# georgegrosu1/torch-admm-deconv

Measured on AMD Instinct MI355X. Metric: ADMM iterations/sec, batch-64 1024x1024x3, 50 iters; rel-L2 vs CPU ref, higher is better.
Workload: dtype f32

## Files before the change

### torch-admm-deconv_amd/csrc/admm_capi.hip

```cpp
#include <hip/hip_runtime.h>

#include <cstdlib>
#include <cstring>
#include <mutex>
#include <string>
#include <type_traits>
#include <vector>

#include "gcol_mm.hpp"
#include "knobs.hpp"
#include "mixed_capi.hpp"
#include "odd_capi.hpp"
#include "admm_tv.h"

using namespace admm;

namespace {

thread_local std::string g_err;

int fail(int code, const std::string& msg) {
    g_err = msg;
    return code;
}
// ... 204 lines not shown
    } while (0)

template <class K> int set_lds(K kern, size_t bytes) {
    if (bytes > 64 * 1024) {
        hipError_t e = hipFuncSetAttribute(reinterpret_cast<const void*>(kern),
                                           hipFuncAttributeMaxDynamicSharedMemorySize, (int)bytes);
        if (e != hipSuccess) return fail(ADMM_TV_EHIP, std::string("hipFuncSetAttribute: ") + hipGetErrorString(e));
    }
    return 0;
}

int launch_check(const char* what) {
    hipError_t e = hipGetLastError();
    if (e != hipSuccess) return fail(ADMM_TV_EHIP, std::string(what) + ": " + hipGetErrorString(e));
    return 0;
}

template <class T>
int bwd_scalars(double* part, int K, long long nstrips, long long spm, long long soff, const double* tpart, int ntp,
                int G, int g, const T* lam, const T* rho, T* glam, T* grho, hipStream_t s) {
    if (K < 1) return fail(ADMM_TV_EINVAL, "bwd_scalars: no iterations");
    hipLaunchKernelGGL(k_bwd_iter_sums, dim3((unsigned)K), dim3(256), 0, s, part, nstrips, spm, soff, tpart, ntp, G, g);
    if (int e = launch_check("k_bwd_iter_sums")) return e;
    hipLaunchKernelGGL(k_bwd_scalars<T>, dim3(1), dim3(256), 0, s, (const double*)part, K, nstrips, 1LL, soff,
                       (const double*)nullptr, ntp, G, g, lam, rho, glam, grho);
    return launch_check("k_bwd_scalars");
}

template <int N> struct RowOps {
    using G = RowKernelGeom<N>;
    static unsigned blocks(long long items) { return (unsigned)((items + G::SG - 1) / G::SG); }

    static int r2c(const float* img, cf* spec, const cf* twW, long long rows, hipStream_t s, bool pl = false) {
        if (pl)
            hipLaunchKernelGGL((k_row_r2c<N, true>), dim3(blocks(rows)), dim3(G::NT), G::lds_bytes(), s, img, spec, twW, rows);
        else
            hipLaunchKernelGGL((k_row_r2c<N, false>), dim3(blocks(rows)), dim3(G::NT), G::lds_bytes(), s, img, spec, twW, rows);
        return launch_check("k_row_r2c");
    }
    static int c2r(const cf* spec, float* img, const cf* twW, long long rows, hipStream_t s, bool pl = false) {
        if (pl)
            hipLaunchKernelGGL((k_row_c2r<N, true>), dim3(blocks(rows)), dim3(G::NT), G::lds_bytes(), s, spec, img, twW, rows);
        else
            hipLaunchKernelGGL((k_row_c2r<N, false>), dim3(blocks(rows)), dim3(G::NT), G::lds_bytes(), s, spec, img, twW, rows);
        return launch_check("k_row_c2r");
    }
    static int pair(const float* img, float* out, long long rows, hipStream_t s) {
        hipLaunchKernelGGL(k_row_pair<N>, dim3(blocks(rows)), dim3(G::NT), 0, s, img, out, rows);
        return launch_check("k_row_pair");
    }
    template <bool ISO, bool FIRST, bool HIST, bool PL> static void pa(const PassAArgs& a, unsigned nb, hipStream_t s) {
        hipLaunchKernelGGL((k_pass_a<N, ISO, FIRST, HIST, PL>), dim3(nb), dim3(G::NT), G::lds_bytes(), s, a);
    }
    static int pass_a(const PassAArgs& a, bool iso, bool first, bool hist, hipStream_t s, bool pl = false) {
        const unsigned nb = blocks(a.nstrips);
        const int sel = (iso ? 4 : 0) | (first ? 2 : 0) | (hist ? 1 : 0);
        if (pl && !hist) {
            switch (sel) {
                case 0: pa<false, false, false, true>(a, nb, s); break;
                case 2: pa<false, true, false, true>(a, nb, s); break;
                case 4: pa<true, false, false, true>(a, nb, s); break;
                default: pa<true, true, false, true>(a, nb, s); break;
            }
            return launch_check("k_pass_a");
        }
        switch (sel) {
            case 0: pa<false, false, false, false>(a, nb, s); break;
            case 1: pa<false, false, true, false>(a, nb, s); break;
            case 2: pa<false, true, false, false>(a, nb, s); break;
            case 3: pa<false, true, true, false>(a, nb, s); break;
            case 4: pa<true, false, false, false>(a, nb, s); break;
            case 5: pa<true, false, true, false>(a, nb, s); break;
            case 6: pa<true, true, false, false>(a, nb, s); break;
            default: pa<true, true, true, false>(a, nb, s); break;
        }
        return launch_check("k_pass_a");
    }
    static int iso_norm(const IsoArgs& a, bool first, bool hist, hipStream_t s, bool pl = false) {
        const unsigned nb = blocks(a.nitems);
        if (first && pl)
            hipLaunchKernelGGL((k_iso_norm<N, true, false, true>), dim3(nb), dim3(G::NT), G::lds_bytes(), s, a);
        else if (first)
            hipLaunchKernelGGL((k_iso_norm<N, true, false, false>), dim3(nb), dim3(G::NT), G::lds_bytes(), s, a);
        else if (hist)
            hipLaunchKernelGGL((k_iso_norm<N, false, true, false>), dim3(nb), dim3(G::NT), G::lds_bytes(), s, a);
        else if (pl)
            hipLaunchKernelGGL((k_iso_norm<N, false, false, true>), dim3(nb), dim3(G::NT), G::lds_bytes(), s, a);
        else
            hipLaunchKernelGGL((k_iso_norm<N, false, false, false>), dim3(nb), dim3(G::NT), G::lds_bytes(), s, a);
        return launch_check("k_iso_norm");
    }
    template <bool ISO, bool LASTK, bool FIRSTK> static void bpa(const BwdArgs& a, unsigned nb, hipStream_t s) {
        using BG = BwdGeom<N>;
        hipLaunchKernelGGL((k_bwd_pass_a<N, ISO, LASTK, FIRSTK>), dim3(nb), dim3(BG::NT), BG::lds_bytes(), s, a);
    }
    static int bwd_pass_a(const BwdArgs& a, bool iso, bool lastk, bool firstk, hipStream_t s) {
        const unsigned nb = (unsigned)((a.nstrips + BwdGeom<N>::SG - 1) / BwdGeom<N>::SG);
        const int sel = (iso ? 4 : 0) | (lastk ? 2 : 0) | (firstk ? 1 : 0);
        switch (sel) {
            case 0: bpa<false, false, false>(a, nb, s); break;
            case 1: bpa<false, false, true>(a, nb, s); break;
            case 2: bpa<false, true, false>(a, nb, s); break;
            case 3: bpa<false, true, true>(a, nb, s); break;
            case 4: bpa<true, false, false>(a, nb, s); break;
            case 5: bpa<true, false, true>(a, nb, s); break;
            case 6: bpa<true, true, false>(a, nb, s); break;
            default: bpa<true, true, true>(a, nb, s); break;
        }
        return launch_check("k_bwd_pass_a");
// ... 1100 lines not shown
    {
        ProfScope ps(3, s);
        if (d.kh > 0) {
            float* bb = at<float>(ws, Lo.b);
            if (env_int("ADMM_MIXED_BGEN", 0)) {
                if (int e = gapply<float>(xin, bb, spec[0], Lo, ws, d, 1, s)) return e;
            } else {
                if (int e = hchk(admm_mixed::r2c(N, xin, spec[0], twW, rows, s), "k_row_r2c_m")) return e;
                if (int e = hchk(admm_mixed::pass_b_cm(H, spec[0], at<cf>(ws, Lo.mM), twH, N, P, s), "k_pass_b_m<cm>"))
                    return e;
                if (int e = hchk(admm_mixed::c2r(N, spec[0], bb, twW, rows, s), "k_row_c2r_m")) return e;
            }
            bimg = bb;
        }
        if (int e = hchk(admm_mixed::r2c(N, bimg, spec[0], twW, rows, s), "k_row_r2c_m")) return e;
    }
    const int R = strip_rows_mixed(H, rows, N);
    const int G = ngroups_of(d);
    const int gpm = Lo.ngroups / G;
    for (int g = 0; g < G; ++g) {
    const float* fcM = at<float>(ws, Lo.fcM) + (size_t)g * (2 * N + 1) * H;
    const float* lamg = lam + g;
    const float* rhog = rho + g;
    float* outg = out + (size_t)g * P * H * W;
    if (g > 0) {
        ProfScope ps(3, s);
        if (int e = hchk(admm_mixed::r2c(N, bimg, spec[0], twW, rows, s), "k_row_r2c_m")) return e;
    }
    int cur = 0, uin = 0;
    for (int it = 1; it <= d.maxit; ++it) {
        {
            ProfScope ps(1, s);
            if (int e = hchk(admm_mixed::pass_b(H, spec[cur], fcM, twH, N, P, s), "k_pass_b_m")) return e;
        }
        if (it == d.maxit) {
            ProfScope ps(3, s);
            if (int e = hchk(admm_mixed::c2r(N, spec[cur], outg, twW, rows, s), "k_row_c2r_m")) return e;
            if (!train) break;
        }
        const bool first = it == 1;
        const float *uxi, *uyi, *nprev = nullptr;
        float *uxo, *uyo;
        if (train) {
            uxi = first ? nullptr : ha(it - 1, 0);
            uyi = first ? nullptr : ha(it - 1, 1);
            uxo = ha(it, 0);
            uyo = ha(it, 1);
            if (d.iso && !first) nprev = hn(it - 1);
        } else {
            uxi = u[2 * uin];
            uyi = u[2 * uin + 1];
            uxo = u[2 * (1 - uin)];
            uyo = u[2 * (1 - uin) + 1];
        }
        const float* nsq = nullptr;
        if (d.iso) {
            ProfScope ps(2, s);
            float* nout = train ? hn(it) : at<float>(ws, Lo.nsq);
            IsoArgs ia{spec[cur], uxi, uyi, nprev, lamg, rhog, at<float>(ws, Lo.part), twW, (int)P, H, Lo.ppg,
                       (long long)gpm * H, P};
            if (int e = hchk(admm_mixed::iso_norm(N, ia, first, train, s), "k_iso_norm_m")) return e;
            const long long n4 = 2LL * H * W / 4;
            hipLaunchKernelGGL(k_iso_reduce, dim3((unsigned)((n4 + 255) / 256)), dim3(256), 0, s, at<float4>(ws, Lo.part),
                               reinterpret_cast<float4*>(nout), gpm, n4);
            if (int e = launch_check("k_iso_reduce")) return e;
            allreduce(d, nout, 2ull * H * W, s);
            nsq = nout;
        }
        {
            ProfScope ps(0, s);
            PassAArgs pa{spec[cur], spec[1 - cur], bimg, uxi, uyi, uxo, uyo, nsq, nprev, lamg, rhog, twW, H, R,
                         rows / R, P, 0};
            if (int e = hchk(admm_mixed::pass_a(N, pa, d.iso != 0, first, train, s), "k_pass_a_m")) return e;
        }
        cur = 1 - cur;
        uin = 1 - uin;
    }
    }
    return 0;
}

int run_forward(const admm_tv_desc& d, const float* xin, const float* kern, const float* lam, const float* rho,
                float* out, void* ws, size_t ws_bytes, void* hist, hipStream_t s) {
    const Layout Lo = make_layout(d);
    if (!ws || ws_bytes < Lo.total || (reinterpret_cast<uintptr_t>(ws) % kAlign) != 0)
        return fail(ADMM_TV_EWORKSPACE, "workspace too small or not 256-byte aligned");
    if (Lo.tr && !hist && d.maxit > 0) {
        const long long P = d.B * d.C;
        const int H = (int)d.H, W = (int)d.W;
        float* xT = at<float>(ws, Lo.xT);
        float* oT = at<float>(ws, Lo.oT);
        float* kT = d.kh > 0 ? at<float>(ws, Lo.kT) : nullptr;
        {
            ProfScope ps(3, s);
            hipError_t e = admm_odd::transpose(xin, xT, H, W, P, s);
            if (e == hipSuccess && kT) e = admm_odd::transpose(kern, kT, d.kh, d.kw, 1, s);
            if (e != hipSuccess) return fail(ADMM_TV_EHIP, std::string("k_transpose: ") + hipGetErrorString(e));
        }
        const admm_tv_desc dT = transposed(d);
        if (int e = run_forward(dT, xT, kT, lam, rho, oT, at<char>(ws, Lo.tws), ws_bytes - Lo.tws, nullptr, s)) return e;
        ProfScope ps(3, s);
        const hipError_t e = admm_odd::transpose(oT, out, W, H, P, s);
        return e == hipSuccess ? 0 : fail(ADMM_TV_EHIP, std::string("k_transpose: ") + hipGetErrorString(e));
    }
    const int G = ngroups_of(d);
    const long long Pm = d.B * d.C, P = G * Pm;
// ... 13 lines not shown
                allreduce(d, at<float>(ws, Lo.nsq), n, s);
            }
        return 0;
    }
    if (int e = setup(d, Lo, ws, kern, rho, s)) return e;
    if (Lo.mixed && (!hist || Lo.mixed_train)) return run_forward_mixed(d, Lo, xin, lam, rho, out, ws, hist, s);
    if (Lo.gen) return run_forward_gen(d, Lo, xin, lam, rho, out, ws, hist, s);
    cf* twW = at<cf>(ws, Lo.twW);
    cf* twH = at<cf>(ws, Lo.twH);
    float* fcT = at<float>(ws, Lo.fcT);
    cf* mT = at<cf>(ws, Lo.mT);
    cf* spec[2] = {at<cf>(ws, Lo.spec[0]), at<cf>(ws, Lo.spec[1])};
    float* u[4] = {at<float>(ws, Lo.u[0]), at<float>(ws, Lo.u[1]), at<float>(ws, Lo.u[2]), at<float>(ws, Lo.u[3])};
    const bool train = hist != nullptr;
    const Hist Hs = make_hist(d);
    auto ha = [&](int k, int comp) -> float* {
        return reinterpret_cast<float*>(static_cast<char*>(hist) + (size_t)(2 * (k - 1) + comp) * Hs.a_slot);
    };
    auto hn = [&](int k) -> float* {
        return reinterpret_cast<float*>(static_cast<char*>(hist) + Hs.n_off + (size_t)(k - 1) * Hs.n_slot);
    };
    const bool keep_t = train && Hs.keep_t;
    auto ht = [&](int k) -> cf* {
        return reinterpret_cast<cf*>(static_cast<char*>(hist) + Hs.t_off + (size_t)(k - 1) * Hs.t_slot);
    };

    const bool pl = !train && env_int("ADMM_PL", (d.iso || W < 1024) ? 1 : 0) != 0;

    const float* bimg = xin;
    if (d.kh > 0) {
        ProfScope ps(3, s);
        float* bb = at<float>(ws, Lo.b);
        if (int e = psf_transpose_into(d, Lo, ws, xin, bb, spec[0], 1, s, pl)) return e;
        bimg = bb;
    } else if (pl) {
        ProfScope ps(3, s);
        float* bb = at<float>(ws, Lo.b);
        if (int e = with_row(N, [&](auto ops) { return decltype(ops)::pair(xin, bb, Pm * H, s); })) return e;
        bimg = bb;
    }
    for (int g = 0; g < G; ++g) {
        ProfScope ps(3, s);
        cf* t0 = (keep_t ? ht(1) : spec[0]) + (size_t)g * Pm * H * N;
        int e = with_row(N, [&](auto ops) { return decltype(ops)::r2c(bimg, t0, twW, Pm * H, s, pl); });
        if (e) return e;
    }
    auto solve_planes = [&](long long p0, long long np, long long ppm, hipStream_t st) -> int {
    const size_t so = (size_t)p0 * H * N, io = (size_t)p0 * H * W;
    cf* cspec[2] = {spec[0] + so, spec[1] + so};
    const long long crows = np * H;
    const float* cb = bimg + io;
    float* cout = out + io;
    const int R = strip_rows(H, N, crows, !d.iso && !hist);

    int cur = 0, uin = 0;
    for (int it = 1; it <= d.maxit; ++it) {
        {
            ProfScope ps(1, st);
            const cf* tin = keep_t ? ht(it) : cspec[cur];
            if (int e = pass_b_oop(H, tin, cspec[cur], fcT, mT, twH, N, (int)np, 0, st, (int)ppm)) return e;
        }
        if (it == d.maxit) {
            ProfScope ps(3, st);
            int e = with_row(N, [&](auto ops) { return decltype(ops)::c2r(cspec[cur], cout, twW, crows, st); });
            if (e) return e;
            if (!train) break;
        }
        const bool first = (it == 1);
        const float *uxi, *uyi, *nprev = nullptr;
        float *uxo, *uyo;
        if (train) {
            uxi = first ? nullptr : ha(it - 1, 0);
            uyi = first ? nullptr : ha(it - 1, 1);
            uxo = ha(it, 0);
            uyo = ha(it, 1);
            if (d.iso && !first) nprev = hn(it - 1);
        } else {
            uxi = u[2 * uin] + io;
            uyi = u[2 * uin + 1] + io;
            uxo = u[2 * (1 - uin)] + io;
            uyo = u[2 * (1 - uin) + 1] + io;
        }
        const float* nsq = nullptr;
        if (d.iso) {
            ProfScope ps(2, st);
            float* nout = train ? hn(it) : at<float>(ws, Lo.nsq);
            IsoArgs ia{cspec[cur], uxi, uyi, nprev, lam, rho, at<float>(ws, Lo.part), twW, (int)P, H, Lo.ppg,
                       (long long)Lo.ngroups * H, Pm};
            int e = with_row(N, [&](auto ops) { return decltype(ops)::iso_norm(ia, first, train, st, pl); });
            if (e) return e;
            const long long n4 = 2LL * H * W / 4;
            const int gpm = Lo.ngroups / G;
            for (int g = 0; g < G; ++g) {
                hipLaunchKernelGGL(k_iso_reduce, dim3((unsigned)((n4 + 255) / 256)), dim3(256), 0, st,
                                   at<float4>(ws, Lo.part) + (size_t)g * gpm * n4,
                                   reinterpret_cast<float4*>(nout) + (size_t)g * n4, gpm, n4);
                if ((e = launch_check("k_iso_reduce"))) return e;
            }
            allreduce(d, nout, (size_t)G * 2 * H * W, st);
            nsq = nout;
        }
        {
            ProfScope ps(0, st);
            cf* tout = (keep_t && it < d.maxit) ? ht(it + 1) : cspec[1 - cur];
            PassAArgs pa{cspec[cur], tout, cb, uxi, uyi, uxo, uyo, nsq, nprev, lam, rho, twW, H, R, crows / R, ppm,
                         env_int("ADMM_PASSA_REV", 0)};
            int e = with_row(N, [&](auto ops) { return decltype(ops)::pass_a(pa, d.iso != 0, first, train, st, pl); });
            if (e) return e;
        }
        cur = 1 - cur;
        uin = 1 - uin;
    }
    return 0;
    };
    return solve_planes(0, P, Pm, s);
}

struct BwdLayout {
    Layout f;
    size_t abar[4], bbar, part, tpart, q, xpart, aacc, zacc, total;
    long long nstrips;
    int R, ntp, xgroups, xppg;
};
BwdLayout make_bwd_layout(const admm_tv_desc& d) {
    BwdLayout B{};
    B.f = make_layout(d);
    const size_t rs = is_f64(d) ? sizeof(double) : sizeof(float);
    const size_t G = ngroups_of(d);
    const size_t img = G * d.B * d.C * d.H * d.W * rs;
    size_t o = B.f.total;
    auto take = [&](size_t bytes) {
        size_t at_ = o;
        o += up(bytes);
        return at_;
    };
    for (int i = 0; i < 4; ++i) B.abar[i] = take(img);
    B.bbar = take(img);
    const long long rows = (long long)G * d.B * d.C * d.H;
    if (B.f.mixed_train) {
        B.R = strip_rows_mixed((int)d.H, rows, (int)d.W / 2, 512);
        B.nstrips = rows / B.R;
    } else if (B.f.gen) {
        B.R = 0;
        B.nstrips = (rows * d.W + 255) / 256;
    } else {
        B.R = strip_rows((int)d.H, (int)d.W / 2, rows);
        B.nstrips = rows / B.R;
    }
    B.part = take((size_t)std::max(d.maxit, 1) * B.nstrips * 2 * sizeof(double));
    B.ntp = (int)std::max<long long>(1, ((long long)d.H * d.W / 2 + 255) / 256);
    B.tpart = take((size_t)std::max(d.maxit, 1) * G * B.ntp * sizeof(double));
    B.q = take(G * 2 * (size_t)d.H * d.W * rs);
    if (d.kh > 0 && (d.flags & ADMM_TV_FLAG_PSF_GRAD)) {
        const size_t nf = ((size_t)d.W / 2 + 1) * d.H;
        B.xppg = 8;
        B.xgroups = (int)((d.B * d.C + B.xppg - 1) / B.xppg);
        B.xpart = take((B.f.gen ? (size_t)d.B * d.C : (size_t)B.xgroups) * nf * 2 * rs);
        B.aacc = take(nf * sizeof(double2));
        B.zacc = take(nf * sizeof(double2));
    }
// ... 571 lines not shown
```

### torch-admm-deconv_amd/csrc/admm_kernels.hpp

```cpp
#pragma once
#include "fft_core.hpp"

namespace admm {

template <int N, class Cfg = RowCfg<N>> struct RowXf {
    static constexpr int E = Cfg::E;
    static constexpr int L = N / E;
    static constexpr int W = 2 * N;
    static_assert(L <= 64, "row transforms keep one row inside one wave");

    __device__ __forceinline__ static void partner(const cf (&v)[E], cf (&p)[E], int t) {
        const int src = (L - t) & (L - 1);
#pragma unroll
        for (int j = 0; j < E; ++j) {
            float a = __shfl(v[E - 1 - j].x, src, L);
            float b = __shfl(v[E - 1 - j].y, src, L);
            p[j] = (t == 0) ? v[(E - j) & (E - 1)] : mkc(a, b);
        }
    }

    __device__ __forceinline__ static void c2r(cf (&v)[E], const RowBuf& buf, const cf* __restrict__ tw, int t) {
        cf p[E];
        partner(v, p, t);
#pragma unroll
// ... 466 lines not shown
    fft<H, L, -1, 1, 1>(v1, buf, tw, t);
#pragma unroll
    for (int j = 0; j < E; ++j) v1[j] = cscale(v1[j], m1[j]);
    fft<H, L, +1, 1, 1>(v1, buf, tw, t);
#pragma unroll
    for (int j = 0; j < E; ++j) bstore_f4(ro, voff, j * sstep, make_float4(v0[j].x, v0[j].y, v1[j].x, v1[j].y));
}

struct PassAArgs {
    const cf* sin;
    cf* sout;
    const float* b;
    const float* uxi;
    const float* uyi;
    float* uxo;
    float* uyo;
    const float* nsq;
    const float* nsq_prev;
    const float* lam;
    const float* rho;
    const cf* twW;
    int H;
    int R;
    long long nstrips;
    long long ppm;
    int rev = 0;
};

#ifndef PASSA_MINW_SMALL
#define PASSA_MINW_SMALL 3
#endif
#define PASSA_MINW(n) ((n) >= 1024 ? 1 : PASSA_MINW_SMALL)

template <bool ISO, class T> __device__ __forceinline__ T shrink_z(T a, T tau, T nsum) {
    if constexpr (ISO) return block_factor(nsum, tau) * a;
    else return soft(a, tau);
}

template <bool ISO, bool FIRST, bool HIST>
__device__ __forceinline__ cf prev_u(const cf* __restrict__ src, const cf* __restrict__ nsp, size_t idx, float tau) {
    if constexpr (FIRST) {
        return mkc(0.f, 0.f);
    } else {
        const cf v = lda<16>(&src[idx]);
        if constexpr (HIST) {
            const cf n = ISO ? nsp[idx] : mkc(0.f, 0.f);
            return mkc(v.x - shrink_z<ISO>(v.x, tau, n.x), v.y - shrink_z<ISO>(v.y, tau, n.y));
        } else {
            return v;
        }
    }
}

template <int N, bool ISO, bool FIRST, bool HIST, bool PL>
__global__ void __launch_bounds__(256, PASSA_MINW(N)) k_pass_a(PassAArgs a) {
    static_assert(!(PL && HIST), "the training history keeps the pixel-order layout");
    using G = RowKernelGeom<N>;
    constexpr int E = G::E, L = G::L, W = G::W;
    constexpr bool kSpecNT = (ADMM_NT & 2) != 0 || ((ADMM_NT & 32) != 0 && N >= 512);
    extern __shared__ __attribute__((aligned(16))) unsigned char smem[];
    cf* tw = reinterpret_cast<cf*>(smem);
    load_tw(tw, a.twW, W);
    __syncthreads();
    const int sgl = threadIdx.x / L, t = threadIdx.x % L;
#ifndef ADMM_PASSA_REMAP
#define ADMM_PASSA_REMAP -1
#endif
    constexpr bool kRemap = ADMM_PASSA_REMAP < 0 ? N <= 256 : ADMM_PASSA_REMAP != 0;
    const unsigned blk = kRemap ? xcd_remap(blockIdx.x, gridDim.x) : blockIdx.x;
    long long strip = (long long)blk * G::SG + sgl;
    if (strip >= a.nstrips) return;
    if (a.rev) strip = a.nstrips - 1 - strip;
    const int H = a.H, R = a.R;
    const int spp = H / R;
    const long long p = strip / spp;
    const int i0 = (int)(strip % spp) * R;
    RowBuf buf{tw + W + sgl * RowBuf::slots(N)};
    const int mod = (int)(p / a.ppm);
    const float rho = a.rho[mod];
    const float tau = a.lam[mod] / rho;

    const cf* sp = a.sin + (size_t)p * H * N;
    cf* so = a.sout + (size_t)p * H * N;
    const size_t poff = (size_t)p * H * W;
    const cf* bimg = reinterpret_cast<const cf*>(a.b + (size_t)(p - (long long)mod * a.ppm) * H * W);
    const cf* uxi = reinterpret_cast<const cf*>(a.uxi + poff);
    const cf* uyi = reinterpret_cast<const cf*>(a.uyi + poff);
    cf* uxo = reinterpret_cast<cf*>(a.uxo + poff);
    cf* uyo = reinterpret_cast<cf*>(a.uyo + poff);
    const size_t moff = (size_t)mod * 2 * H * W;
    const cf* nsx = reinterpret_cast<const cf*>(a.nsq + moff);
    const cf* nsy = reinterpret_cast<const cf*>(a.nsq + moff + (size_t)H * W);
    const cf* npx = reinterpret_cast<const cf*>(a.nsq_prev + moff);
    const cf* npy = reinterpret_cast<const cf*>(a.nsq_prev + moff + (size_t)H * W);

    cf xprev[E], xcur[E], wxp[E], wyp[E];
    {
        const int g = (i0 - 1 + H) & (H - 1);
#pragma unroll
        for (int j = 0; j < E; ++j) xprev[j] = ld_pol<kSpecNT>(&sp[(size_t)g * N + t + L * j]);
        RowXf<N>::c2r(xprev, buf, tw, t);
    }
    for (int rr = 0; rr <= R; ++rr) {
        const int g = (i0 + rr) & (H - 1);
        const size_t ro = (size_t)g * N;
#pragma unroll
        for (int j = 0; j < E; ++j) xcur[j] = ld_pol<kSpecNT>(&sp[ro + t + L * j]);
        RowXf<N>::c2r(xcur, buf, tw, t);

        cf wyc[E];
        {
            cf uy[E], fy[E];
            if constexpr (PL) {
                if constexpr (FIRST) {
#pragma unroll
                    for (int j = 0; j < E; ++j) uy[j] = mkc(0.f, 0.f);
                } else {
                    ld_row<E, L, true, (ADMM_NT & 16) != 0>(uyi + ro, t, uy);
                }
                if constexpr (ISO) ld_row<E, L, true, false>(nsy + ro, t, fy);
            } else {
#pragma unroll
                for (int j = 0; j < E; ++j) {
                    uy[j] = prev_u<ISO, FIRST, HIST>(uyi, npy, ro + t + L * j, tau);
                    if constexpr (ISO) fy[j] = nsy[ro + t + L * j];
                }
            }
#pragma unroll
            for (int j = 0; j < E; ++j) {
                const float a0 = (xcur[j].x - xprev[j].x) + uy[j].x;
                const float a1 = (xcur[j].y - xprev[j].y) + uy[j].y;
                const float z0 = shrink_z<ISO>(a0, tau, ISO ? fy[j].x : 0.f);
                const float z1 = shrink_z<ISO>(a1, tau, ISO ? fy[j].y : 0.f);
                const float n0 = a0 - z0, n1 = a1 - z1;
                uy[j] = HIST ? mkc(a0, a1) : mkc(n0, n1);
                wyc[j] = mkc(z0 - n0, z1 - n1);
            }
            if (rr < R) {
                if constexpr (PL) {
                    st_row<E, L, true, (ADMM_NT & 1) != 0>(uyo + ro, t, uy);
                } else {
#pragma unroll
                    for (int j = 0; j < E; ++j) sta(&uyo[ro + t + L * j], uy[j]);
                }
            }
        }

        if (rr >= 1) {
            const int gm = (g - 1 + H) & (H - 1);
            const size_t rm = (size_t)gm * N;
            cf r[E], sh[E], bv[E];
            if constexpr (PL) ld_row<E, L, true, (ADMM_NT & 16) != 0>(bimg + rm, t, bv);
#pragma unroll
            for (int j = 0; j < E; ++j) sh[j].x = __shfl(wxp[j].x, (t + 1) & (L - 1), L);
#pragma unroll
            for (int j = 0; j < E; ++j) {
                const float wr = (t == L - 1) ? sh[(j + 1) & (E - 1)].x : sh[j].x;
                const cf bb = PL ? bv[j] : lda<16>(&bimg[rm + t + L * j]);
                const float v0 = (wxp[j].x - wxp[j].y) + (wyp[j].x - wyc[j].x);
                const float v1 = (wxp[j].y - wr) + (wyp[j].y - wyc[j].y);
                r[j] = mkc(fmaf(rho, v0, bb.x), fmaf(rho, v1, bb.y));
            }
            RowXf<N>::r2c(r, buf, tw, t);
#pragma unroll
            for (int j = 0; j < E; ++j) sta(&so[rm + t + L * j], r[j]);
        }

        if (rr < R) {
            cf ux[E], fx[E], sh[E];
            if constexpr (PL) {
                if constexpr (FIRST) {
#pragma unroll
                    for (int j = 0; j < E; ++j) ux[j] = mkc(0.f, 0.f);
                } else {
                    ld_row<E, L, true, (ADMM_NT & 16) != 0>(uxi + ro, t, ux);
                }
                if constexpr (ISO) ld_row<E, L, true, false>(nsx + ro, t, fx);
            }
#pragma unroll
            for (int j = 0; j < E; ++j) {
                if constexpr (!PL) {
                    ux[j] = prev_u<ISO, FIRST, HIST>(uxi, npx, ro + t + L * j, tau);
                    if constexpr (ISO) fx[j] = nsx[ro + t + L * j];
                }
                sh[j].x = __shfl(xcur[j].y, (t - 1) & (L - 1), L);
            }
#pragma unroll
            for (int j = 0; j < E; ++j) {
                const float xl = (t == 0) ? sh[(j - 1) & (E - 1)].x : sh[j].x;
                const float a0 = (xcur[j].x - xl) + ux[j].x;
                const float a1 = (xcur[j].y - xcur[j].x) + ux[j].y;
                const float z0 = shrink_z<ISO>(a0, tau, ISO ? fx[j].x : 0.f);
                const float z1 = shrink_z<ISO>(a1, tau, ISO ? fx[j].y : 0.f);
                const float n0 = a0 - z0, n1 = a1 - z1;
                ux[j] = HIST ? mkc(a0, a1) : mkc(n0, n1);
                wxp[j] = mkc(z0 - n0, z1 - n1);
            }
            if constexpr (PL) {
                st_row<E, L, true, (ADMM_NT & 1) != 0>(uxo + ro, t, ux);
            } else {
#pragma unroll
                for (int j = 0; j < E; ++j) sta(&uxo[ro + t + L * j], ux[j]);
            }
        }
#pragma unroll
        for (int j = 0; j < E; ++j) {
            wyp[j] = wyc[j];
            xprev[j] = xcur[j];
        }
    }
}

struct IsoArgs {
    const cf* sin;
    const float* uxi;
    const float* uyi;
    const float* nsq_prev;
    const float* lam;
    const float* rho;
    float* partial;
    const cf* twW;
    int P, H, ppg;
    long long nitems;
    long long ppm;
};

template <int N, bool FIRST, bool HIST, bool PL>
__global__ void __launch_bounds__(256) k_iso_norm(IsoArgs a) {
    static_assert(!(PL && HIST), "the training history keeps the pixel-order layout");
    using G = RowKernelGeom<N>;
    constexpr int E = G::E, L = G::L, W = G::W;
    extern __shared__ __attribute__((aligned(16))) unsigned char smem[];
    cf* tw = reinterpret_cast<cf*>(smem);
    load_tw(tw, a.twW, W);
    __syncthreads();
    const int sgl = threadIdx.x / L, t = threadIdx.x % L;
    const long long item = (long long)blockIdx.x * G::SG + sgl;
    if (item >= a.nitems) return;
    const int H = a.H;
    const int g = (int)(item % H);
    const int grp = (int)(item / H);
    const int gm = (g - 1 + H) & (H - 1);
    RowBuf buf{tw + W + sgl * RowBuf::slots(N)};
    const int mod = (int)((long long)grp * a.ppg / a.ppm);
    const float tau = HIST ? a.lam[mod] / a.rho[mod] : 0.f;
    const size_t moff = (size_t)mod * 2 * H * W;
    const cf* npx = reinterpret_cast<const cf*>(a.nsq_prev + moff);
    const cf* npy = reinterpret_cast<const cf*>(a.nsq_prev + moff + (size_t)H * W);
    cf sx[E], sy[E];
#pragma unroll
    for (int j = 0; j < E; ++j) sx[j] = sy[j] = mkc(0.f, 0.f);
    const int p1 = min(a.P, (grp + 1) * a.ppg);
    for (int p = grp * a.ppg; p < p1; ++p) {
        const cf* sp = a.sin + (size_t)p * H * N;
        cf xp[E], xc[E];
#pragma unroll
        for (int j = 0; j < E; ++j) {
            xp[j] = sp[(size_t)gm * N + t + L * j];
            xc[j] = sp[(size_t)g * N + t + L * j];
        }
        RowXf<N>::c2r(xp, buf, tw, t);
        RowXf<N>::c2r(xc, buf, tw, t);
// ... 60 lines not shown
```

### torch-admm-deconv_amd/csrc/mixed_kernels.hpp

```cpp
#pragma once
#include <type_traits>

#include "admm_backward.hpp"
#include "admm_kernels.hpp"
#include "mixed_fft.hpp"

namespace admm {

template <int N, int L> __host__ __device__ constexpr bool edge_ok(int R, int Lx) {
    return ((N / R + L - 1) / L == 1 && N / R == Lx) || (L == Lx && (N / R) % L == 0);
}
template <int N> struct MRow;
template <int N> struct MRowPow2 {
    static constexpr int Lg = N / RowCfg<N>::E, Lp = Lg, Ls = Lg, Ep = RowCfg<N>::E, Es = Ep;
    using Inv = typename RowCfg<N>::S;
    using Fwd = typename RowCfg<N>::S;
};
template <> struct MRow<16> : MRowPow2<16> {};
template <> struct MRow<32> : MRowPow2<32> {};
template <> struct MRow<64> : MRowPow2<64> {};
template <> struct MRow<128> : MRowPow2<128> {};
template <> struct MRow<256> : MRowPow2<256> {};
template <> struct MRow<512> : MRowPow2<512> {};
template <> struct MRow<1024> {
// ... 544 lines not shown
#pragma unroll
    for (int j = 0; j < Ec; ++j) bstore_cf(rs, voff, j * sstep, v[j]);
}

#ifdef ADMM_PASSA_M_W
#define PASSA_M_MINW(ep) (ADMM_PASSA_M_W)
#else
#define PASSA_M_MINW(ep) ((ep) > 9 ? 1 : 2)
#endif
#ifndef ADMM_TRAIN_FWD_PLAN
#define ADMM_TRAIN_FWD_PLAN 1
#endif
template <int N> constexpr bool train_fwd_plan() {
    return ADMM_TRAIN_FWD_PLAN == 2 || (ADMM_TRAIN_FWD_PLAN == 1 && MRowT<N>::Lg == MRow<N>::Lg);
}
#ifndef ADMM_INFER_TPLAN
#define ADMM_INFER_TPLAN 1
#endif
template <int N> constexpr bool infer_tplan() { return ADMM_INFER_TPLAN != 0 && MRowT<N>::Lg == MRow<N>::Lg; }
template <int N, bool TRAIN>
using MPlan = typename std::conditional<TRAIN ? train_fwd_plan<N>() : infer_tplan<N>(), MRowT<N>, MRow<N>>::type;
template <int N, bool ISO, bool FIRST, bool HIST>
__global__ void __launch_bounds__(256, PASSA_M_MINW((MPlan<N, HIST>::Ep))) k_pass_a_m(PassAArgs a) {
    using G = MRowG<N, MPlan<N, HIST>>;
    using Xf = RowXfM<N, MPlan<N, HIST>>;
    constexpr int Lg = G::Lg, Lp = G::Lp, Ep = G::Ep, Ls = G::Ls, Es = G::Es, EM = G::EM, W = G::W;
    constexpr bool kSpecNT = (ADMM_NT & 2) != 0 || ((ADMM_NT & 32) != 0 && N >= 512);
    constexpr bool kUNT = (ADMM_NT & 16) != 0;
    extern __shared__ __attribute__((aligned(16))) unsigned char smem[];
    cf* tw = reinterpret_cast<cf*>(smem);
    load_tw(tw, a.twW, W);
    __syncthreads();
    const int sgl = threadIdx.x / Lg, t = threadIdx.x % Lg;
    long long strip = (long long)blockIdx.x * G::SG + sgl;
    const bool ok = strip < a.nstrips;
    if (!G::WIDE && !ok) return;
    if (!ok) strip = a.nstrips - 1;
    const int H = a.H, R = a.R;
    const int spp = H / R;
    const long long p = strip / spp;
    const int i0 = (int)(strip % spp) * R;
    auto lx = Xf::lds_of(tw + W + sgl * RowBuf::slots(N));
    const float rho = a.rho[0];
    const float tau = a.lam[0] / rho;
    const bool pa = t < Lp, sa = t < Ls;
    const bool pst = ok && pa, sst = ok && sa;

    const cf* sp = a.sin + (size_t)p * H * N;
    cf* so = a.sout + (size_t)p * H * N;
    const size_t poff = (size_t)p * H * W;
    const cf* bimg = reinterpret_cast<const cf*>(a.b + poff);
    const cf* uxi = reinterpret_cast<const cf*>(a.uxi + poff);
    const cf* uyi = reinterpret_cast<const cf*>(a.uyi + poff);
    cf* uxo = reinterpret_cast<cf*>(a.uxo + poff);
    cf* uyo = reinterpret_cast<cf*>(a.uyo + poff);
    const cf* nsx = reinterpret_cast<const cf*>(a.nsq);
    const cf* nsy = reinterpret_cast<const cf*>(a.nsq + (size_t)H * W);
    const cf* npx = reinterpret_cast<const cf*>(a.nsq_prev);
    const cf* npy = reinterpret_cast<const cf*>(a.nsq_prev + (size_t)H * W);

    auto xrow = [&](int g, cf (&x)[Ep]) {
        cf v[EM];
        if (sa) {
#pragma unroll
            for (int j = 0; j < Es; ++j) v[j] = ld_pol<kSpecNT>(&sp[(size_t)g * N + t + Ls * j]);
        }
        Xf::c2r(v, lx, tw, t);
#pragma unroll
        for (int j = 0; j < Ep; ++j) x[j] = v[j];
    };
    cf xprev[Ep], xcur[Ep], wxp[Ep], wyp[Ep];
    xrow(i0 == 0 ? H - 1 : i0 - 1, xprev);
    for (int rr = 0; rr <= R; ++rr) {
        const int g = i0 + rr >= H ? i0 + rr - H : i0 + rr;
        const size_t ro = (size_t)g * N;
        xrow(g, xcur);

        cf wyc[Ep];
        {
            cf uy[Ep], fy[Ep];
#pragma unroll
            for (int j = 0; j < Ep; ++j) {
                if constexpr (HIST) uy[j] = pa ? prev_u<ISO, FIRST, true>(uyi, npy, ro + t + Lp * j, tau) : mkc(0.f, 0.f);
                else uy[j] = (FIRST || !pa) ? mkc(0.f, 0.f) : ld_pol<kUNT>(&uyi[ro + t + Lp * j]);
                if constexpr (ISO) fy[j] = pa ? nsy[ro + t + Lp * j] : mkc(0.f, 0.f);
            }
#pragma unroll
            for (int j = 0; j < Ep; ++j) {
                const float a0 = (xcur[j].x - xprev[j].x) + uy[j].x;
                const float a1 = (xcur[j].y - xprev[j].y) + uy[j].y;
                const float z0 = shrink_z<ISO>(a0, tau, ISO ? fy[j].x : 0.f);
                const float z1 = shrink_z<ISO>(a1, tau, ISO ? fy[j].y : 0.f);
                const float n0 = a0 - z0, n1 = a1 - z1;
                uy[j] = HIST ? mkc(a0, a1) : mkc(n0, n1);
                wyc[j] = mkc(z0 - n0, z1 - n1);
            }
            if (rr < R && pst) {
#pragma unroll
                for (int j = 0; j < Ep; ++j) sta(&uyo[ro + t + Lp * j], uy[j]);
            }
        }

        if (rr >= 1) {
            const int gm = g == 0 ? H - 1 : g - 1;
            const size_t rm = (size_t)gm * N;
            float wxs[Ep], wrs[Ep];
#pragma unroll
            for (int j = 0; j < Ep; ++j) wxs[j] = wxp[j].x;
            Xf::template neighbour<+1>(wxs, wrs, lx, t);
            cf r[EM];
#pragma unroll
            for (int j = 0; j < Ep; ++j) {
                const float wr = wrs[j];
                const cf bb = pa ? lda<16>(&bimg[rm + t + Lp * j]) : mkc(0.f, 0.f);
                const float v0 = (wxp[j].x - wxp[j].y) + (wyp[j].x - wyc[j].x);
                const float v1 = (wxp[j].y - wr) + (wyp[j].y - wyc[j].y);
                r[j] = mkc(fmaf(rho, v0, bb.x), fmaf(rho, v1, bb.y));
            }
            Xf::r2c(r, lx, tw, t);
            if (sst) {
#pragma unroll
                for (int j = 0; j < Es; ++j) sta(&so[rm + t + Ls * j], r[j]);
            }
        }

        if (rr < R) {
            cf ux[Ep], fx[Ep];
            float xys[Ep], xls[Ep];
#pragma unroll
            for (int j = 0; j < Ep; ++j) {
                if constexpr (HIST) ux[j] = pa ? prev_u<ISO, FIRST, true>(uxi, npx, ro + t + Lp * j, tau) : mkc(0.f, 0.f);
                else ux[j] = (FIRST || !pa) ? mkc(0.f, 0.f) : ld_pol<kUNT>(&uxi[ro + t + Lp * j]);
                if constexpr (ISO) fx[j] = pa ? nsx[ro + t + Lp * j] : mkc(0.f, 0.f);
                xys[j] = xcur[j].y;
            }
            Xf::template neighbour<-1>(xys, xls, lx, t);
#pragma unroll
            for (int j = 0; j < Ep; ++j) {
                const float xl = xls[j];
                const float a0 = (xcur[j].x - xl) + ux[j].x;
                const float a1 = (xcur[j].y - xcur[j].x) + ux[j].y;
                const float z0 = shrink_z<ISO>(a0, tau, ISO ? fx[j].x : 0.f);
                const float z1 = shrink_z<ISO>(a1, tau, ISO ? fx[j].y : 0.f);
                const float n0 = a0 - z0, n1 = a1 - z1;
                ux[j] = HIST ? mkc(a0, a1) : mkc(n0, n1);
                wxp[j] = mkc(z0 - n0, z1 - n1);
            }
            if (pst) {
#pragma unroll
                for (int j = 0; j < Ep; ++j) sta(&uxo[ro + t + Lp * j], ux[j]);
            }
        }
#pragma unroll
        for (int j = 0; j < Ep; ++j) {
            wyp[j] = wyc[j];
            xprev[j] = xcur[j];
        }
    }
}

template <int N, bool FIRST, bool HIST>
__global__ void __launch_bounds__(256) k_iso_norm_m(IsoArgs a) {
    using G = MRowG<N, MPlan<N, HIST>>;
    using Xf = RowXfM<N, MPlan<N, HIST>>;
    constexpr int Lg = G::Lg, Lp = G::Lp, Ep = G::Ep, Ls = G::Ls, Es = G::Es, EM = G::EM, W = G::W;
    extern __shared__ __attribute__((aligned(16))) unsigned char smem[];
    cf* tw = reinterpret_cast<cf*>(smem);
    load_tw(tw, a.twW, W);
    __syncthreads();
    const int sgl = threadIdx.x / Lg, t = threadIdx.x % Lg;
    long long item = (long long)blockIdx.x * G::SG + sgl;
    const bool ok = item < a.nitems;
    if (!G::WIDE && !ok) return;
    if (!ok) item = a.nitems - 1;
    const int H = a.H;
    const int g = (int)(item % H);
    const int grp = (int)(item / H);
    const int gm = g == 0 ? H - 1 : g - 1;
    auto lx = Xf::lds_of(tw + W + sgl * RowBuf::slots(N));
    const bool pa = t < Lp, sa = t < Ls;
    const float tau = HIST ? a.lam[0] / a.rho[0] : 0.f;
    const cf* npx = reinterpret_cast<const cf*>(a.nsq_prev);
    const cf* npy = reinterpret_cast<const cf*>(a.nsq_prev + (size_t)H * W);
    cf sx[Ep], sy[Ep];
#pragma unroll
    for (int j = 0; j < Ep; ++j) sx[j] = sy[j] = mkc(0.f, 0.f);
    const int p1 = min(a.P, (grp + 1) * a.ppg);
    for (int p = grp * a.ppg; p < p1; ++p) {
        const cf* sp = a.sin + (size_t)p * H * N;
        cf vp[EM], vc[EM];
        if (sa) {
#pragma unroll
            for (int j = 0; j < Es; ++j) {
                vp[j] = sp[(size_t)gm * N + t + Ls * j];
                vc[j] = sp[(size_t)g * N + t + Ls * j];
            }
        }
        Xf::c2r(vp, lx, tw, t);
        Xf::c2r(vc, lx, tw, t);
        const size_t ro = (size_t)p * H * N + (size_t)g * N;
        const cf* uxi = reinterpret_cast<const cf*>(a.uxi);
// ... 336 lines not shown
```

Before: 708.7.

## Add cooperative row-pass strips sharing boundary rows via LDS; skip final dual stores

For N=512 anisotropic inference, adds a cooperative variant of the row pass. Pairs of waves in a block walk a strip from opposite ends and exchange boundary rows and y-direction weights through an LDS mailbox. This removes the redundant halo-row inverse transform each strip otherwise recomputes, at the cost of extra LDS, barriers and more complex control flow. Separately, on the second-to-last iteration the dual-variable stores are skipped by passing null output pointers, since those duals are never read again.

```diff
diff --git a/torch-admm-deconv_amd/csrc/admm_capi.hip b/torch-admm-deconv_amd/csrc/admm_capi.hip
--- a/torch-admm-deconv_amd/csrc/admm_capi.hip
+++ b/torch-admm-deconv_amd/csrc/admm_capi.hip
@@ -280,9 +280,22 @@
     template <bool ISO, bool FIRST, bool HIST, bool PL> static void pa(const PassAArgs& a, unsigned nb, hipStream_t s) {
         hipLaunchKernelGGL((k_pass_a<N, ISO, FIRST, HIST, PL>), dim3(nb), dim3(G::NT), G::lds_bytes(), s, a);
     }
-    static int pass_a(const PassAArgs& a, bool iso, bool first, bool hist, hipStream_t s, bool pl = false) {
+    static constexpr bool kCoop = N == 512;
+    template <bool FIRST, bool PL> static void pa_coop(const PassAArgs& a, unsigned nb, hipStream_t s) {
+        if constexpr (kCoop)
+            hipLaunchKernelGGL((k_pass_a<N, false, FIRST, false, PL, true>), dim3(nb), dim3(G::NT), passa_coop_lds<N>(), s, a);
+    }
+    static int pass_a(const PassAArgs& a, bool iso, bool first, bool hist, hipStream_t s, bool pl = false,
+                      bool coop = false) {
         const unsigned nb = blocks(a.nstrips);
         const int sel = (iso ? 4 : 0) | (first ? 2 : 0) | (hist ? 1 : 0);
+        if (kCoop && coop && !iso && !hist && !a.rev && a.R >= 2 && a.nstrips % G::SG == 0 &&
+            (a.H / a.R) % G::SG == 0) {
+            static_assert(!kCoop || passa_coop_lds<N>() <= 53 * 1024, "three blocks of the row pass per CU");
+            if (first) pl ? pa_coop<true, true>(a, nb, s) : pa_coop<true, false>(a, nb, s);
+            else pl ? pa_coop<false, true>(a, nb, s) : pa_coop<false, false>(a, nb, s);
+            return launch_check("k_pass_a");
+        }
         if (pl && !hist) {
             switch (sel) {
                 case 0: pa<false, false, false, true>(a, nb, s); break;
@@ -1489,6 +1502,7 @@
             uyi = u[2 * uin + 1];
             uxo = u[2 * (1 - uin)];
             uyo = u[2 * (1 - uin) + 1];
+            if (it == d.maxit - 1) uxo = uyo = nullptr;
         }
         const float* nsq = nullptr;
         if (d.iso) {
@@ -1608,6 +1622,7 @@
     const float* cb = bimg + io;
     float* cout = out + io;
     const int R = strip_rows(H, N, crows, !d.iso && !hist);
+    const bool coop = env_int("ADMM_PASSA_COOP", 1) != 0;
 
     int cur = 0, uin = 0;
     for (int it = 1; it <= d.maxit; ++it) {
@@ -1636,6 +1651,7 @@
             uyi = u[2 * uin + 1] + io;
             uxo = u[2 * (1 - uin)] + io;
             uyo = u[2 * (1 - uin) + 1] + io;
+            if (it == d.maxit - 1) uxo = uyo = nullptr;
         }
         const float* nsq = nullptr;
         if (d.iso) {
@@ -1661,7 +1677,9 @@
             cf* tout = (keep_t && it < d.maxit) ? ht(it + 1) : cspec[1 - cur];
             PassAArgs pa{cspec[cur], tout, cb, uxi, uyi, uxo, uyo, nsq, nprev, lam, rho, twW, H, R, crows / R, ppm,
                          env_int("ADMM_PASSA_REV", 0)};
-            int e = with_row(N, [&](auto ops) { return decltype(ops)::pass_a(pa, d.iso != 0, first, train, st, pl); });
+            int e = with_row(N, [&](auto ops) {
+                return decltype(ops)::pass_a(pa, d.iso != 0, first, train, st, pl, coop);
+            });
             if (e) return e;
         }
         cur = 1 - cur;
diff --git a/torch-admm-deconv_amd/csrc/admm_kernels.hpp b/torch-admm-deconv_amd/csrc/admm_kernels.hpp
--- a/torch-admm-deconv_amd/csrc/admm_kernels.hpp
+++ b/torch-admm-deconv_amd/csrc/admm_kernels.hpp
@@ -542,25 +542,31 @@
     }
 }
 
-template <int N, bool ISO, bool FIRST, bool HIST, bool PL>
+template <int N> constexpr size_t passa_coop_lds() {
+    return RowKernelGeom<N>::lds_bytes() + sizeof(cf) * (RowKernelGeom<N>::SG - 1) * N;
+}
+template <int N, bool ISO, bool FIRST, bool HIST, bool PL, bool COOP = false>
 __global__ void __launch_bounds__(256, PASSA_MINW(N)) k_pass_a(PassAArgs a) {
     static_assert(!(PL && HIST), "the training history keeps the pixel-order layout");
     using G = RowKernelGeom<N>;
-    constexpr int E = G::E, L = G::L, W = G::W;
+    constexpr int E = G::E, L = G::L, W = G::W, SG = G::SG;
+    static_assert(!COOP || (L == 64 && SG % 2 == 0 && !HIST && !ISO), "cooperative strips: whole waves in pairs, aniso inference");
     constexpr bool kSpecNT = (ADMM_NT & 2) != 0 || ((ADMM_NT & 32) != 0 && N >= 512);
     extern __shared__ __attribute__((aligned(16))) unsigned char smem[];
     cf* tw = reinterpret_cast<cf*>(smem);
     load_tw(tw, a.twW, W);
     __syncthreads();
-    const int sgl = threadIdx.x / L, t = threadIdx.x % L;
+    const int sgl = COOP ? __builtin_amdgcn_readfirstlane(threadIdx.x / L) : threadIdx.x / L, t = threadIdx.x % L;
 #ifndef ADMM_PASSA_REMAP
 #define ADMM_PASSA_REMAP -1
 #endif
     constexpr bool kRemap = ADMM_PASSA_REMAP < 0 ? N <= 256 : ADMM_PASSA_REMAP != 0;
     const unsigned blk = kRemap ? xcd_remap(blockIdx.x, gridDim.x) : blockIdx.x;
     long long strip = (long long)blk * G::SG + sgl;
-    if (strip >= a.nstrips) return;
-    if (a.rev) strip = a.nstrips - 1 - strip;
+    if constexpr (!COOP) {
+        if (strip >= a.nstrips) return;
+        if (a.rev) strip = a.nstrips - 1 - strip;
+    }
     const int H = a.H, R = a.R;
     const int spp = H / R;
     const long long p = strip / spp;
@@ -576,29 +582,22 @@
     const cf* bimg = reinterpret_cast<const cf*>(a.b + (size_t)(p - (long long)mod * a.ppm) * H * W);
     const cf* uxi = reinterpret_cast<const cf*>(a.uxi + poff);
     const cf* uyi = reinterpret_cast<const cf*>(a.uyi + poff);
-    cf* uxo = reinterpret_cast<cf*>(a.uxo + poff);
-    cf* uyo = reinterpret_cast<cf*>(a.uyo + poff);
+    const bool ust = HIST || a.uxo != nullptr;
+    cf* uxo = ust ? reinterpret_cast<cf*>(a.uxo + poff) : nullptr;
+    cf* uyo = ust ? reinterpret_cast<cf*>(a.uyo + poff) : nullptr;
     const size_t moff = (size_t)mod * 2 * H * W;
     const cf* nsx = reinterpret_cast<const cf*>(a.nsq + moff);
     const cf* nsy = reinterpret_cast<const cf*>(a.nsq + moff + (size_t)H * W);
     const cf* npx = reinterpret_cast<const cf*>(a.nsq_prev + moff);
     const cf* npy = reinterpret_cast<const cf*>(a.nsq_prev + moff + (size_t)H * W);
 
-    cf xprev[E], xcur[E], wxp[E], wyp[E];
-    {
-        const int g = (i0 - 1 + H) & (H - 1);
-#pragma unroll
-        for (int j = 0; j < E; ++j) xprev[j] = ld_pol<kSpecNT>(&sp[(size_t)g * N + t + L * j]);
-        RowXf<N>::c2r(xprev, buf, tw, t);
-    }
-    for (int rr = 0; rr <= R; ++rr) {
-        const int g = (i0 + rr) & (H - 1);
+    auto xrow = [&](int g, cf (&x)[E]) __attribute__((always_inline)) {
+#pragma unroll
+        for (int j = 0; j < E; ++j) x[j] = ld_pol<kSpecNT>(&sp[(size_t)g * N + t + L * j]);
+        RowXf<N>::c2r(x, buf, tw, t);
+    };
+    auto ydir = [&](int g, const cf (&xg)[E], const cf (&xup)[E], bool store, cf (&wyc)[E]) __attribute__((always_inline)) {
         const size_t ro = (size_t)g * N;
-#pragma unroll
-        for (int j = 0; j < E; ++j) xcur[j] = ld_pol<kSpecNT>(&sp[ro + t + L * j]);
-        RowXf<N>::c2r(xcur, buf, tw, t);
-
-        cf wyc[E];
         {
             cf uy[E], fy[E];
             if constexpr (PL) {
@@ -618,15 +617,15 @@
             }
 #pragma unroll
             for (int j = 0; j < E; ++j) {
-                const float a0 = (xcur[j].x - xprev[j].x) + uy[j].x;
-                const float a1 = (xcur[j].y - xprev[j].y) + uy[j].y;
+                const float a0 = (xg[j].x - xup[j].x) + uy[j].x;
+                const float a1 = (xg[j].y - xup[j].y) + uy[j].y;
                 const float z0 = shrink_z<ISO>(a0, tau, ISO ? fy[j].x : 0.f);
                 const float z1 = shrink_z<ISO>(a1, tau, ISO ? fy[j].y : 0.f);
                 const float n0 = a0 - z0, n1 = a1 - z1;
                 uy[j] = HIST ? mkc(a0, a1) : mkc(n0, n1);
                 wyc[j] = mkc(z0 - n0, z1 - n1);
             }
-            if (rr < R) {
+            if (store && ust) {
                 if constexpr (PL) {
                     st_row<E, L, true, (ADMM_NT & 1) != 0>(uyo + ro, t, uy);
                 } else {
@@ -635,9 +634,9 @@
                 }
             }
         }
-
-        if (rr >= 1) {
-            const int gm = (g - 1 + H) & (H - 1);
+    };
+    auto finish = [&](int gm, const cf (&wxp)[E], const cf (&wyp)[E], const cf (&wyc)[E]) __attribute__((always_inline)) {
+        {
             const size_t rm = (size_t)gm * N;
             cf r[E], sh[E], bv[E];
             if constexpr (PL) ld_row<E, L, true, (ADMM_NT & 16) != 0>(bimg + rm, t, bv);
@@ -655,8 +654,10 @@
 #pragma unroll
             for (int j = 0; j < E; ++j) sta(&so[rm + t + L * j], r[j]);
         }
-
-        if (rr < R) {
+    };
+    auto xdir = [&](int g, const cf (&xcur)[E], cf (&wxp)[E]) __attribute__((always_inline)) {
+        const size_t ro = (size_t)g * N;
+        {
             cf ux[E], fx[E], sh[E];
             if constexpr (PL) {
                 if constexpr (FIRST) {
@@ -686,18 +687,91 @@
                 ux[j] = HIST ? mkc(a0, a1) : mkc(n0, n1);
                 wxp[j] = mkc(z0 - n0, z1 - n1);
             }
-            if constexpr (PL) {
-                st_row<E, L, true, (ADMM_NT & 1) != 0>(uxo + ro, t, ux);
-            } else {
-#pragma unroll
-                for (int j = 0; j < E; ++j) sta(&uxo[ro + t + L * j], ux[j]);
-            }
-        }
+            if (ust) {
+                if constexpr (PL) {
+                    st_row<E, L, true, (ADMM_NT & 1) != 0>(uxo + ro, t, ux);
+                } else {
+#pragma unroll
+                    for (int j = 0; j < E; ++j) sta(&uxo[ro + t + L * j], ux[j]);
+                }
+            }
+        }
+    };
+
+    cf xprev[E], xcur[E], wxp[E], wyp[E], wyc[E];
+    auto pick = [](bool c, cf p, cf q) __attribute__((always_inline)) { return mkc(c ? p.x : q.x, c ? p.y : q.y); };
+    auto ystep = [&](bool up, int gy, bool store) __attribute__((always_inline)) {
+        cf xg[E], xup[E];
+#pragma unroll
+        for (int j = 0; j < E; ++j) {
+            xg[j] = pick(up, xprev[j], xcur[j]);
+            xup[j] = pick(up, xcur[j], xprev[j]);
+        }
+        ydir(gy, xg, xup, store, wyc);
+    };
+    auto fstep = [&](bool up, int gf) __attribute__((always_inline)) {
+        cf wa[E], wb[E];
+#pragma unroll
+        for (int j = 0; j < E; ++j) {
+            wa[j] = pick(up, wyc[j], wyp[j]);
+            wb[j] = pick(up, wyp[j], wyc[j]);
+        }
+        finish(gf, wxp, wa, wb);
+    };
+    auto shift = [&]() __attribute__((always_inline)) {
 #pragma unroll
         for (int j = 0; j < E; ++j) {
             wyp[j] = wyc[j];
             xprev[j] = xcur[j];
         }
+    };
+    auto step = [&](bool up, int g, bool ystore, bool fin, bool xd) __attribute__((always_inline)) {
+        xrow(g, xcur);
+        const int gn = up ? (g + 1) & (H - 1) : g;
+        ystep(up, gn, ystore);
+        if (fin) fstep(up, up ? gn : (g - 1 + H) & (H - 1));
+        if (xd) xdir(g, xcur, wxp);
+        shift();
+    };
+    if constexpr (!COOP) {
+        xrow((i0 - 1 + H) & (H - 1), xprev);
+        for (int rr = 0; rr <= R; ++rr) step(false, (i0 + rr) & (H - 1), rr < R, rr >= 1, rr < R);
+    } else {
+        cf* mbox = tw + W + SG * RowBuf::slots(N);
+        const bool up = (sgl & 1) != 0, top = sgl == 0, bot = sgl == SG - 1;
+        cf* mbs = mbox + (size_t)min(max(up ? sgl : sgl - 1, 0), SG - 2) * N;
+        cf* mbe = mbox + (size_t)(up ? sgl - 1 : sgl) * N;
+        auto put = [&](cf* mb, const cf (&v)[E]) __attribute__((always_inline)) {
+#pragma unroll
+            for (int j = 0; j < E; ++j) mb[t + L * j] = v[j];
+        };
+        auto get = [&](const cf* mb, cf (&v)[E]) __attribute__((always_inline)) {
+#pragma unroll
+            for (int j = 0; j < E; ++j) v[j] = mb[t + L * j];
+        };
+        const int gs = up ? i0 + R - 1 : i0;
+        if (top || bot) xrow((top ? i0 - 1 + H : i0 + R) & (H - 1), xprev);
+        xrow(gs, xcur);
+        if (up && !bot) put(mbs, xcur);
+        lds_barrier();
+        if (!up && !top) get(mbs, xprev);
+        if (!up || bot) ystep(up, up ? (i0 + R) & (H - 1) : gs, !up);
+        if (!up && !top) put(mbs, wyc);
+        lds_barrier();
+        if (up && !bot) get(mbs, wyc);
+        xdir(gs, xcur, wxp);
+        shift();
+        for (int rr = 1; rr < R; ++rr) step(up, up ? i0 + R - 1 - rr : i0 + rr, true, true, true);
+        if (!up) put(mbe, xprev);
+        lds_barrier();
+        if (up) {
+            get(mbe, xcur);
+            ystep(true, i0, true);
+            put(mbe, wyc);
+        }
+        lds_barrier();
+        if (!up) get(mbe, wyc);
+        fstep(up, up ? i0 : i0 + R - 1);
     }
 }
 
diff --git a/torch-admm-deconv_amd/csrc/mixed_kernels.hpp b/torch-admm-deconv_amd/csrc/mixed_kernels.hpp
--- a/torch-admm-deconv_amd/csrc/mixed_kernels.hpp
+++ b/torch-admm-deconv_amd/csrc/mixed_kernels.hpp
@@ -620,8 +620,9 @@
     const cf* bimg = reinterpret_cast<const cf*>(a.b + poff);
     const cf* uxi = reinterpret_cast<const cf*>(a.uxi + poff);
     const cf* uyi = reinterpret_cast<const cf*>(a.uyi + poff);
-    cf* uxo = reinterpret_cast<cf*>(a.uxo + poff);
-    cf* uyo = reinterpret_cast<cf*>(a.uyo + poff);
+    const bool ust = HIST || a.uxo != nullptr;
+    cf* uxo = ust ? reinterpret_cast<cf*>(a.uxo + poff) : nullptr;
+    cf* uyo = ust ? reinterpret_cast<cf*>(a.uyo + poff) : nullptr;
     const cf* nsx = reinterpret_cast<const cf*>(a.nsq);
     const cf* nsy = reinterpret_cast<const cf*>(a.nsq + (size_t)H * W);
     const cf* npx = reinterpret_cast<const cf*>(a.nsq_prev);
@@ -663,7 +664,7 @@
                 uy[j] = HIST ? mkc(a0, a1) : mkc(n0, n1);
                 wyc[j] = mkc(z0 - n0, z1 - n1);
             }
-            if (rr < R && pst) {
+            if (rr < R && pst && ust) {
 #pragma unroll
                 for (int j = 0; j < Ep; ++j) sta(&uyo[ro + t + Lp * j], uy[j]);
             }
@@ -714,7 +715,7 @@
                 ux[j] = HIST ? mkc(a0, a1) : mkc(n0, n1);
                 wxp[j] = mkc(z0 - n0, z1 - n1);
             }
-            if (pst) {
+            if (pst && ust) {
 #pragma unroll
                 for (int j = 0; j < Ep; ++j) sta(&uxo[ro + t + Lp * j], ux[j]);
             }
```

New measurement: 722.3 (median of 6 runs). 1.02x the previous value.
